# yewsiang/Transferable3D

Hardware: AMD Instinct MI355X
Metric: frustums/sec fwd+bwd (higher is better)
Workload: dtype f32

## Files before the change

### transferable3d_amd/csrc/poolbwd.hip

```cpp
#include "poolbwd_dev.h"

namespace {

__global__ __launch_bounds__(256) void k_pool_bwd_prep(const t3d_pool_bwd_prep_args p) {
  extern __shared__ __attribute__((aligned(16))) float smem[];
  pool_bwd_prep_body(p, smem, blockIdx.x, blockIdx.y, blockIdx.z);
}
__global__ __launch_bounds__(256) void k_pool_sparse_rows(const t3d_pool_sparse_rows_args p) {
  extern __shared__ __attribute__((aligned(16))) float smem[];
  pool_sparse_rows_body(p, smem, blockIdx.x, blockIdx.y);
}
template <class XT>
__global__ __launch_bounds__(256) void k_act_colsum(const t3d_act_colsum_args p) {
  extern __shared__ __attribute__((aligned(16))) float smem[];
  act_colsum_body<XT>(p, smem, blockIdx.x);
}
template <class XT>
__global__ __launch_bounds__(256) void k_pool_wgrad_finish(const t3d_pool_wgrad_finish_args p) {
  extern __shared__ __attribute__((aligned(16))) float smem[];
  pool_wgrad_finish_body<XT>(p, smem, blockIdx.x, blockIdx.y);
}

}

extern "C" int t3d_pool_bwd_prep(const t3d_pool_bwd_prep_args* a, t3d_stream_t stream) {
  const int rc = check_prep(a);
  if (rc != T3D_OK) return rc;
  T3D_LAUNCH(k_pool_bwd_prep, dim3(a->K / 32, a->K / 32, (a->N + PCH - 1) / PCH), dim3(256), PREP_LDS,
             static_cast<hipStream_t>(stream), *a);
  T3D_CHECK_LAUNCH();
  return T3D_OK;
}

extern "C" int t3d_pool_sparse_rows(const t3d_pool_sparse_rows_args* a, t3d_stream_t stream) {
  const int rc = check_sparse_rows(a);
  if (rc != T3D_OK) return rc;
  const size_t lds = sparse_rows_lds(a->N);
  static size_t allowed = 0;
  if (lds > 64 * 1024 && lds > allowed) {
    (void)hipFuncSetAttribute(reinterpret_cast<const void*>(k_pool_sparse_rows), hipFuncAttributeMaxDynamicSharedMemorySize,
                              (int)lds);
    allowed = lds;
  }
  const long M = (long)a->B * a->rows_per_frustum;
  T3D_LAUNCH(k_pool_sparse_rows, dim3(M / 128, a->K / SR_KC), dim3(256), lds, static_cast<hipStream_t>(stream), *a);
  T3D_CHECK_LAUNCH();
  return T3D_OK;
}

extern "C" int t3d_act_colsum(const t3d_act_colsum_args* a, t3d_stream_t stream) {
  const int rc = check_colsum(a);
  if (rc != T3D_OK) return rc;
  if (a->a.dtype == T3D_BF16) T3D_LAUNCH(k_act_colsum<bf16_t>, dim3(a->M / 128), dim3(256), COLSUM_LDS, static_cast<hipStream_t>(stream), *a);
  else T3D_LAUNCH(k_act_colsum<float>, dim3(a->M / 128), dim3(256), COLSUM_LDS, static_cast<hipStream_t>(stream), *a);
  T3D_CHECK_LAUNCH();
  return T3D_OK;
}

extern "C" int t3d_pool_wgrad_finish(const t3d_pool_wgrad_finish_args* a, t3d_stream_t stream) {
  const int rc = check_finish(a);
  if (rc != T3D_OK) return rc;
  const size_t lds = finish_lds(a->K);
  if (a->a.dtype == T3D_BF16) T3D_LAUNCH(k_pool_wgrad_finish<bf16_t>, dim3(a->K / FK, a->N / FN), dim3(256), lds, static_cast<hipStream_t>(stream), *a);
  else T3D_LAUNCH(k_pool_wgrad_finish<float>, dim3(a->K / FK, a->N / FN), dim3(256), lds, static_cast<hipStream_t>(stream), *a);
  T3D_CHECK_LAUNCH();
  return T3D_OK;
}
```

### transferable3d_amd/csrc/poolbwd_dev.h

```cpp
#pragma once
#include "common.h"

namespace {


constexpr int PCH = 128;

constexpr size_t PREP_LDS = (2 * 32 * (PCH + 1) + 2 * PCH) * sizeof(float);

__device__ __forceinline__ void pool_bwd_prep_body(const t3d_pool_bwd_prep_args& p, float* smem, int bi, int bj, int ch, int tid_ = -1) {
  float (*wi)[PCH + 1] = reinterpret_cast<float (*)[PCH + 1]>(smem);
  float (*wj)[PCH + 1] = reinterpret_cast<float (*)[PCH + 1]>(smem + 32 * (PCH + 1));
  float* v = smem + 2 * 32 * (PCH + 1);
  float* c0s = v + PCH;
  const int tid = tid_ < 0 ? (int)threadIdx.x : tid_, ti = tid >> 4, tj = tid & 15;
  const int n0 = ch * PCH;
  const bool edge = bj == 0;
  const float* c0 = p.coef;
  const float* c1 = p.coef + p.N;
  const float* c2 = p.coef + 2 * p.N;
#pragma unroll
  for (int q = 0; q < 4; ++q) {
    const int f = tid + 256 * q;
    const int r = f >> 5, c = (f & 31) * 4;
    const int n = min(n0 + c, p.N - 4);
    const bool ok = n0 + c < p.N;
    const float4 a = *reinterpret_cast<const float4*>(p.w + (size_t)(32 * bi + r) * p.N + n);
    const float4 b = *reinterpret_cast<const float4*>(p.w + (size_t)(32 * bj + r) * p.N + n);
    const float4 s1 = *reinterpret_cast<const float4*>(c1 + n);
    wi[r][c + 0] = ok ? a.x : 0.f; wi[r][c + 1] = ok ? a.y : 0.f; wi[r][c + 2] = ok ? a.z : 0.f; wi[r][c + 3] = ok ? a.w : 0.f;
    wj[r][c + 0] = ok ? b.x * s1.x : 0.f; wj[r][c + 1] = ok ? b.y * s1.y : 0.f;
    wj[r][c + 2] = ok ? b.z * s1.z : 0.f; wj[r][c + 3] = ok ? b.w * s1.w : 0.f;
  }
  if (tid < PCH) {
    const int n = min(n0 + tid, p.N - 1);
    const bool ok = n0 + tid < p.N;
    v[tid] = ok ? fmaf(p.bias ? p.bias[n] : 0.f, c1[n], c2[n]) : 0.f;
    c0s[tid] = ok ? c0[n] : 0.f;
  }
  __syncthreads();
  float a00 = 0.f, a01 = 0.f, a10 = 0.f, a11 = 0.f;
#pragma unroll 8
  for (int c = 0; c < PCH; ++c) {
    const float x0 = wi[ti][c], x1 = wi[ti + 16][c], y0 = wj[tj][c], y1 = wj[tj + 16][c];
    a00 = fmaf(x0, y0, a00); a01 = fmaf(x0, y1, a01);
    a10 = fmaf(x1, y0, a10); a11 = fmaf(x1, y1, a11);
  }
  float* ps = p.p_slabs + (size_t)ch * p.K * p.K;
  ps[(size_t)(32 * bi + ti) * p.K + 32 * bj + tj] = a00;
  ps[(size_t)(32 * bi + ti) * p.K + 32 * bj + tj + 16] = a01;
  ps[(size_t)(32 * bi + ti + 16) * p.K + 32 * bj + tj] = a10;
  ps[(size_t)(32 * bi + ti + 16) * p.K + 32 * bj + tj + 16] = a11;
  if (edge) {
    const int r = tid >> 3, q = tid & 7;
    float rc = 0.f;
#pragma unroll
    for (int c = q; c < PCH; c += 8) rc = fmaf(wi[r][c], v[c], rc);
    rc += __shfl_xor(rc, 4, 64);
    rc += __shfl_xor(rc, 2, 64);
    rc += __shfl_xor(rc, 1, 64);
    if (q == 0) p.rc_slabs[(size_t)ch * p.K + 32 * bi + r] = rc;
    const int k = tid & 31;
    if (p.wc != nullptr)
      for (int c = tid >> 5; c < PCH; c += 8)
        if (n0 + c < p.N) p.wc[(size_t)(n0 + c) * p.K + 32 * bi + k] = c0s[c] * wi[k][c];
  }
}

constexpr int SR_KC = 128;
constexpr int SR_UNROLL = 16;
constexpr int SR_PRE = 16;

__device__ __forceinline__ void pool_sparse_rows_body(const t3d_pool_sparse_rows_args& p, float* smem, int bx, int by) {
  float* tile = smem;
  int* lists = reinterpret_cast<int*>(smem + 128 * SR_KC);
  int* hitrow = lists + 4 * p.N;
  const int tid = threadIdx.x, lane = tid & 63, w = tid >> 6;
  const int row0 = bx * 128, kc0 = by * SR_KC;
  const int b = row0 / p.rows_per_frustum, rin0 = row0 - b * p.rows_per_frustum;
  for (int f = tid; f < 128 * SR_KC / 4; f += 256) reinterpret_cast<float4*>(tile)[f] = make_float4(0.f, 0.f, 0.f, 0.f);
  if (tid < 128) hitrow[tid] = 0;
  int* mine = lists + w * p.N;
  int cnt = 0;
  for (int nb = 0; nb < p.N; nb += 64 * SR_PRE) {
    int rr[SR_PRE];
#pragma unroll
    for (int q = 0; q < SR_PRE; ++q) {
      const int n = nb + 64 * q + lane;
      rr[q] = p.argidx[(size_t)b * p.N + min(n, p.N - 1)];
    }
#pragma unroll
    for (int q = 0; q < SR_PRE; ++q) {
      const int n = nb + 64 * q + lane;
      const int r = rr[q] - rin0;
      const bool hit = n < p.N && r >= 0 && r < 128 && (r & 3) == w;
      const unsigned long long m = __ballot(hit);
      if (hit) mine[cnt + __popcll(m & ((1ull << lane) - 1ull))] = n | (r << 16);
      cnt += __popcll(m);
    }
  }
  __syncthreads();
  for (int i0 = 0; i0 < cnt; i0 += SR_UNROLL) {
    float2 wv[SR_UNROLL];
    float g[SR_UNROLL];
    int rr[SR_UNROLL], en[SR_UNROLL];
#pragma unroll
    for (int u = 0; u < SR_UNROLL; ++u) en[u] = mine[min(i0 + u, cnt - 1)];
#pragma unroll
    for (int u = 0; u < SR_UNROLL; ++u) {
      const int n = en[u] & 0xffff;
      rr[u] = en[u] >> 16;
      g[u] = p.dpool[(size_t)b * p.N + n];
      wv[u] = *reinterpret_cast<const float2*>(p.wc + (size_t)n * p.K + kc0 + 2 * lane);
    }
#pragma unroll
    for (int u = 0; u < SR_UNROLL; ++u) {
      hitrow[rr[u]] = 1;
      g[u] = (i0 + u < cnt) ? g[u] : 0.f;
    }
#pragma unroll
    for (int u = 0; u < SR_UNROLL; ++u) {
      float2* t = reinterpret_cast<float2*>(tile + rr[u] * SR_KC + 2 * lane);
      float2 cur = *t;
      cur.x = fmaf(g[u], wv[u].x, cur.x);
      cur.y = fmaf(g[u], wv[u].y, cur.y);
      *t = cur;
    }
  }
  __syncthreads();
  const bool gated = p.row_live != nullptr;
  if (gated && by == 0 && tid < 128) p.row_live[row0 + tid] = hitrow[tid];
  for (int f = tid; f < 128 * SR_KC / 4; f += 256) {
    const int r = f / (SR_KC / 4), c4 = f % (SR_KC / 4);
    if (gated && !hitrow[r]) continue;
    *reinterpret_cast<float4*>(p.s + (size_t)(row0 + r) * p.K + kc0 + 4 * c4) = reinterpret_cast<const float4*>(tile)[f];
  }
}

__device__ __forceinline__ float act_elem(const t3d_act_src& s, size_t row, int k) {
  float v = ld_elem(s.x, row * s.ldx + s.coff + k, s.dtype);
  if (s.scale) v = fmaf(v, s.scale[k], s.shift[k]);
  if (s.relu) v = fmaxf(v, 0.f);
  return v;
}

constexpr size_t COLSUM_LDS = 256 * sizeof(float4);

template <class XT = float>
__device__ __forceinline__ void act_colsum_body(const t3d_act_colsum_args& p, float* smem, int bx) {
  float4* red = reinterpret_cast<float4*>(smem);
  const int tid = threadIdx.x;
  const int row0 = bx * 128;
  const int chunks = p.K / 4, c4 = tid % chunks, grp = tid / chunks, groups = 256 / chunks, rows = 128 / groups;
  float4 sc = make_float4(1.f, 1.f, 1.f, 1.f), sh = make_float4(0.f, 0.f, 0.f, 0.f);
  if (p.a.scale) {
    sc = *reinterpret_cast<const float4*>(p.a.scale + 4 * c4);
    sh = *reinterpret_cast<const float4*>(p.a.shift + 4 * c4);
  }
  const float floor_ = p.a.relu ? 0.f : -INFINITY;
  float4 acc = make_float4(0.f, 0.f, 0.f, 0.f);
  const size_t base = (size_t)(row0 + grp * rows) * p.a.ldx + p.a.coff + 4 * c4;
  constexpr int CSB = 16;
  for (int r0 = 0; r0 < rows; r0 += CSB) {
    typename Elem<XT>::V4 raw[CSB];
#pragma unroll
    for (int u = 0; u < CSB; ++u) raw[u] = Elem<XT>::ld4(p.a.x, base + (size_t)min(r0 + u, rows - 1) * p.a.ldx);
#pragma unroll
    for (int u = 0; u < CSB; ++u) {
      if (r0 + u < rows) {
        const float4 x = Elem<XT>::widen(raw[u]);
        acc.x += fmaxf(fmaf(x.x, sc.x, sh.x), floor_);
        acc.y += fmaxf(fmaf(x.y, sc.y, sh.y), floor_);
        acc.z += fmaxf(fmaf(x.z, sc.z, sh.z), floor_);
        acc.w += fmaxf(fmaf(x.w, sc.w, sh.w), floor_);
      }
    }
  }
  red[tid] = acc;
  __syncthreads();
  if (tid < chunks) {
    float4 t = red[tid];
    for (int g = 1; g < groups; ++g) {
      const float4 u = red[g * chunks + tid];
      t.x += u.x; t.y += u.y; t.z += u.z; t.w += u.w;
    }
    *reinterpret_cast<float4*>(p.part + (size_t)bx * p.K + 4 * tid) = t;
  }
}

constexpr int FK = 32, FN = 16, FB = 32;

inline size_t finish_lds(int K) {
  return ((size_t)FK * (K + 1) + (size_t)K * FN + FK * (FN + 1) + 2 * FB * FN) * sizeof(float);
}

template <class XT = float>
__device__ __forceinline__ void pool_wgrad_finish_body(const t3d_pool_wgrad_finish_args& p, float* smem, int bx, int by, int tid_ = -1) {
  float* gsm = smem;
  float* wsm = gsm + FK * (p.K + 1);
  float* gat = wsm + p.K * FN;
  float* dps = gat + FK * (FN + 1);
  int* ais = reinterpret_cast<int*>(dps + FB * FN);
  const int tid = tid_ < 0 ? (int)threadIdx.x : tid_;
  const int k0 = bx * FK, n0 = by * FN;
  const int ldg = p.K + 1;
  for (int f = tid; f < FK * p.K; f += 256) gsm[(f / p.K) * ldg + f % p.K] = p.g[(size_t)(k0 + f / p.K) * p.K + f % p.K];
  for (int f = tid; f < p.K * FN; f += 256) wsm[f] = p.w[(size_t)(f / FN) * p.N + n0 + f % FN];
  {
    const int k = tid & 31, q = tid >> 5;
    const float sc = p.a.scale ? p.a.scale[k0 + k] : 1.f, sh = p.a.scale ? p.a.shift[k0 + k] : 0.f;
    const float floor_ = p.a.relu ? 0.f : -INFINITY;
    const size_t xk = (size_t)(p.a.coff + k0 + k);
    float g0 = 0.f, g1 = 0.f;
    for (int b0 = 0; b0 < p.B; b0 += FB) {
      __syncthreads();
      for (int f = tid; f < FB * FN; f += 256) {
        const int b = b0 + f / FN;
        const bool ok = b < p.B;
        const size_t o = (size_t)min(b, p.B - 1) * p.N + n0 + f % FN;
        const int ai = p.argidx[o];
        const float dpv = p.dpool[o];
        dps[f] = (ok && ai >= 0) ? dpv : 0.f;
        ais[f] = max(ai, 0);
      }
      __syncthreads();
      float x0[FB], x1[FB];
#pragma unroll
      for (int bb = 0; bb < FB; ++bb) {
        const size_t rowbase = (size_t)min(b0 + bb, p.B - 1) * p.rows_per_frustum;
        x0[bb] = Elem<XT>::ld1(p.a.x, xk + (rowbase + ais[bb * FN + q]) * p.a.ldx);
        x1[bb] = Elem<XT>::ld1(p.a.x, xk + (rowbase + ais[bb * FN + q + 8]) * p.a.ldx);
      }
#pragma unroll
      for (int bb = 0; bb < FB; ++bb) {
        g0 = fmaf(dps[bb * FN + q], fmaxf(fmaf(x0[bb], sc, sh), floor_), g0);
        g1 = fmaf(dps[bb * FN + q + 8], fmaxf(fmaf(x1[bb], sc, sh), floor_), g1);
      }
    }
    gat[k * (FN + 1) + q] = g0;
    gat[k * (FN + 1) + q + 8] = g1;
  }
  __syncthreads();
  const int ti = tid >> 4, tj = tid & 15;
  float a0 = 0.f, a1 = 0.f;
#pragma unroll 8
  for (int j = 0; j < p.K; ++j) {
    const float wv = wsm[j * FN + tj];
    a0 = fmaf(gsm[ti * ldg + j], wv, a0);
    a1 = fmaf(gsm[(ti + 16) * ldg + j], wv, a1);
  }
  const int n = n0 + tj;
  const float c0 = p.coef[n], c1 = p.coef[p.N + n], c2 = p.coef[2 * p.N + n];
  const float bias = p.bias ? p.bias[n] : 0.f;
  const float ab0 = p.abar[k0 + ti], ab1 = p.abar[k0 + ti + 16];
  p.dw[(size_t)(k0 + ti) * p.N + n] = fmaf(c0, gat[ti * (FN + 1) + tj], fmaf(c1, fmaf(ab0, bias, a0), ab0 * c2));
  p.dw[(size_t)(k0 + ti + 16) * p.N + n] = fmaf(c0, gat[(ti + 16) * (FN + 1) + tj], fmaf(c1, fmaf(ab1, bias, a1), ab1 * c2));
}



inline bool pool_act_ok(const t3d_act_src& a, int K) {
  return a.x != nullptr && a.coff + K <= a.ldx && (a.scale == nullptr || a.shift != nullptr) && a.sub == nullptr;
}
inline int check_prep(const t3d_pool_bwd_prep_args* a) {
  if (!a || !a->w || !a->coef || !a->p_slabs || !a->rc_slabs) return T3D_ERR_ARG;
  if (a->K <= 0 || a->K % 32 || a->N <= 0 || a->N % 4) return T3D_ERR_SHAPE;
  return T3D_OK;
}
inline size_t sparse_rows_lds(int N) { return (size_t)128 * SR_KC * sizeof(float) + ((size_t)4 * N + 128) * sizeof(int); }
inline int check_sparse_rows(const t3d_pool_sparse_rows_args* a) {
  if (!a || !a->argidx || !a->dpool || !a->wc || !a->s) return T3D_ERR_ARG;
  if (a->B <= 0 || a->N <= 0 || a->N > 65535 || a->K % SR_KC || a->rows_per_frustum % T3D_TILE_ROWS ||
      a->rows_per_frustum > 32767 || sparse_rows_lds(a->N) > 160 * 1024)
    return T3D_ERR_SHAPE;
  return T3D_OK;
}
inline int check_colsum(const t3d_act_colsum_args* a) {
  if (!a || !a->part || !pool_act_ok(a->a, a->K)) return T3D_ERR_ARG;
  if (a->M <= 0 || a->M % T3D_TILE_ROWS || (a->K != 64 && a->K != 128 && a->K != 256) || a->a.ldx % 4 || a->a.coff % 4)
    return T3D_ERR_SHAPE;
  return T3D_OK;
}
inline int check_finish(const t3d_pool_wgrad_finish_args* a) {
  if (!a || !a->argidx || !a->dpool || !a->coef || !a->w || !a->g || !a->abar || !a->dw || !pool_act_ok(a->a, a->K))
    return T3D_ERR_ARG;
  if (a->K <= 0 || a->K % FK || a->K > 256 || a->N <= 0 || a->N % FN || a->B <= 0) return T3D_ERR_SHAPE;
  return T3D_OK;
}

}
```

Before: 27660.

## Rewrite sparse-row pooling backward as counting-sort row lists with segmented accumulation

Replaces the default sparse-rows kernel with a version that buckets hit points by destination row via wave-ballot ranking, a prefix scan over per-wave row counts, and a compact sorted (offset|row, grad) list. Waves then split the sorted list into balanced row-aligned ranges and do a segmented FMA accumulation with double-buffered prefetch of weight rows, writing only touched rows and zeroing empty ones directly. This targets the zero-fill of the full LDS tile and the per-row scanning cost of the old scheme. The old tile kernel stays reachable through an environment variable, and a new shape check guards the 32-bit byte offset packing.

```diff
diff --git a/transferable3d_amd/csrc/poolbwd.hip b/transferable3d_amd/csrc/poolbwd.hip
--- a/transferable3d_amd/csrc/poolbwd.hip
+++ b/transferable3d_amd/csrc/poolbwd.hip
@@ -1,3 +1,4 @@
+#include <stdlib.h>
 #include "poolbwd_dev.h"
 
 namespace {
@@ -9,6 +10,10 @@
 __global__ __launch_bounds__(256) void k_pool_sparse_rows(const t3d_pool_sparse_rows_args p) {
   extern __shared__ __attribute__((aligned(16))) float smem[];
   pool_sparse_rows_body(p, smem, blockIdx.x, blockIdx.y);
+}
+__global__ __launch_bounds__(256) void k_pool_sparse_rows_tile(const t3d_pool_sparse_rows_args p) {
+  extern __shared__ __attribute__((aligned(16))) float smem[];
+  pool_sparse_rows_tile_body(p, smem, blockIdx.x, blockIdx.y);
 }
 template <class XT>
 __global__ __launch_bounds__(256) void k_act_colsum(const t3d_act_colsum_args p) {
@@ -36,14 +41,17 @@
   const int rc = check_sparse_rows(a);
   if (rc != T3D_OK) return rc;
   const size_t lds = sparse_rows_lds(a->N);
-  static size_t allowed = 0;
-  if (lds > 64 * 1024 && lds > allowed) {
-    (void)hipFuncSetAttribute(reinterpret_cast<const void*>(k_pool_sparse_rows), hipFuncAttributeMaxDynamicSharedMemorySize,
-                              (int)lds);
-    allowed = lds;
+  const char* e_ = getenv("T3D_SPARSE_ROWS");
+  const bool tile = e_ && atoi(e_) == 0;
+  static size_t allowed[2] = {0, 0};
+  if (lds > 64 * 1024 && lds > allowed[tile]) {
+    (void)hipFuncSetAttribute(tile ? reinterpret_cast<const void*>(k_pool_sparse_rows_tile) : reinterpret_cast<const void*>(k_pool_sparse_rows),
+                              hipFuncAttributeMaxDynamicSharedMemorySize, (int)lds);
+    allowed[tile] = lds;
   }
   const long M = (long)a->B * a->rows_per_frustum;
-  T3D_LAUNCH(k_pool_sparse_rows, dim3(M / 128, a->K / SR_KC), dim3(256), lds, static_cast<hipStream_t>(stream), *a);
+  if (tile) T3D_LAUNCH(k_pool_sparse_rows_tile, dim3(M / 128, a->K / SR_KC), dim3(256), lds, static_cast<hipStream_t>(stream), *a);
+  else T3D_LAUNCH(k_pool_sparse_rows, dim3(M / 128, a->K / SR_KC), dim3(256), lds, static_cast<hipStream_t>(stream), *a);
   T3D_CHECK_LAUNCH();
   return T3D_OK;
 }
diff --git a/transferable3d_amd/csrc/poolbwd_dev.h b/transferable3d_amd/csrc/poolbwd_dev.h
--- a/transferable3d_amd/csrc/poolbwd_dev.h
+++ b/transferable3d_amd/csrc/poolbwd_dev.h
@@ -70,8 +70,194 @@
 constexpr int SR_KC = 128;
 constexpr int SR_UNROLL = 16;
 constexpr int SR_PRE = 16;
+constexpr int SRL_PRE = 8;
+constexpr int SRL_U = 16;
+constexpr int SRL_OFF = 128 * SR_KC;
+constexpr int SRL_LIST = SRL_OFF + 130;
+
+__device__ __forceinline__ void srl_issue(int2 (&en)[SRL_U], float2 (&wv)[SRL_U], const int2* ent, const char* wcb, unsigned lane8,
+                                          int i0, int e) {
+#pragma unroll
+  for (int u = 0; u < SRL_U; ++u) en[u] = ent[min(i0 + u, e - 1)];
+#pragma unroll
+  for (int u = 0; u < SRL_U; ++u) wv[u] = *reinterpret_cast<const float2*>(wcb + (((unsigned)en[u].x & ~511u) | lane8));
+}
+
+template <bool TAIL>
+__device__ __forceinline__ void srl_consume(const int2 (&en)[SRL_U], const float2 (&wv)[SRL_U], float* rows, int rem, int& prev, float2& acc) {
+#pragma unroll
+  for (int u = 0; u < SRL_U; ++u) {
+    if (!TAIL || u < rem) {
+      const int row = en[u].x & 127;
+      const float g = __int_as_float(en[u].y);
+      const bool fresh = row != prev;
+      acc.x = fmaf(g, wv[u].x, fresh ? 0.f : acc.x);
+      acc.y = fmaf(g, wv[u].y, fresh ? 0.f : acc.y);
+      *reinterpret_cast<float2*>(rows + row * SR_KC) = acc;
+      prev = row;
+    }
+  }
+}
 
 __device__ __forceinline__ void pool_sparse_rows_body(const t3d_pool_sparse_rows_args& p, float* smem, int bx, int by) {
+  int* cnt = reinterpret_cast<int*>(smem);
+  int* stage = cnt + 4 * 128;
+  float* dstage = reinterpret_cast<float*>(stage + p.N);
+  int* off = cnt + SRL_OFF;
+  int2* list = reinterpret_cast<int2*>(cnt + SRL_LIST);
+  const int tid = threadIdx.x, lane = tid & 63;
+  const int w = __builtin_amdgcn_readfirstlane(tid >> 6);
+  const int row0 = bx * 128, kc0 = by * SR_KC;
+  const int b = row0 / p.rows_per_frustum, rin0 = row0 - b * p.rows_per_frustum;
+  const bool gated = p.row_live != nullptr;
+  const int cpw = ((p.N + 63) / 64 + 3) / 4;
+  const int n_lo = min(w * cpw * 64, p.N), n_hi = min(n_lo + cpw * 64, p.N);
+  int* mycnt = cnt + w * 128;
+  mycnt[lane] = 0;
+  mycnt[lane + 64] = 0;
+  for (int nb = n_lo; nb < n_hi; nb += 64 * SRL_PRE) {
+    int rr[SRL_PRE];
+    float dd[SRL_PRE];
+#pragma unroll
+    for (int q = 0; q < SRL_PRE; ++q) {
+      const size_t o = (size_t)b * p.N + min(nb + 64 * q + lane, p.N - 1);
+      rr[q] = p.argidx[o];
+      dd[q] = p.dpool[o];
+    }
+#pragma unroll
+    for (int q = 0; q < SRL_PRE; ++q) {
+      const int n = nb + 64 * q + lane;
+      if (nb + 64 * q < n_hi) {
+        const int r = rr[q] - rin0;
+        const bool hit = n < n_hi && r >= 0 && r < 128;
+        unsigned long long rem = __ballot(hit);
+        int rank = 0, tot = 0, lead = lane;
+        while (rem) {
+          const int l = __ffsll(rem) - 1;
+          const int rl = __builtin_amdgcn_readlane(r, l);
+          const bool me = hit && r == rl;
+          const unsigned long long m = __ballot(me);
+          const int below = __builtin_amdgcn_mbcnt_hi((unsigned)(m >> 32), __builtin_amdgcn_mbcnt_lo((unsigned)m, 0u));
+          rank = me ? below : rank;
+          tot = me ? __popcll(m) : tot;
+          lead = me ? l : lead;
+          rem &= ~m;
+        }
+        int old = 0;
+        if (hit && lead == lane) {
+          old = mycnt[r];
+          mycnt[r] = old + tot;
+        }
+        old = __shfl(old, lead, 64);
+        if (n < n_hi) {
+          stage[n] = hit ? (r << 16) | (old + rank) : -1;
+          dstage[n] = dd[q];
+        }
+      }
+    }
+  }
+  __syncthreads();
+  if (w == 0) {
+    int c0[4], c1[4];
+#pragma unroll
+    for (int q = 0; q < 4; ++q) {
+      const int2 c = *reinterpret_cast<const int2*>(cnt + q * 128 + 2 * lane);
+      c0[q] = c.x;
+      c1[q] = c.y;
+    }
+    const int t0 = c0[0] + c0[1] + c0[2] + c0[3], t1 = c1[0] + c1[1] + c1[2] + c1[3];
+    int incl = t0 + t1;
+#pragma unroll
+    for (int d = 1; d < 64; d <<= 1) {
+      const int v = __shfl_up(incl, d, 64);
+      if (lane >= d) incl += v;
+    }
+    const int excl = incl - (t0 + t1);
+    *reinterpret_cast<int2*>(off + 2 * lane) = make_int2(excl, excl + t0);
+    if (lane == 63) off[128] = incl;
+    int run0 = excl, run1 = excl + t0;
+#pragma unroll
+    for (int q = 0; q < 4; ++q) {
+      *reinterpret_cast<int2*>(cnt + q * 128 + 2 * lane) = make_int2(run0, run1);
+      run0 += c0[q];
+      run1 += c1[q];
+    }
+    if (gated && by == 0) {
+      p.row_live[row0 + 2 * lane] = t0 > 0;
+      p.row_live[row0 + 2 * lane + 1] = t1 > 0;
+    }
+  }
+  __syncthreads();
+  for (int n = n_lo + lane; n < n_hi; n += 64) {
+    const int e = stage[n];
+    if (e >= 0) {
+      const int r = e >> 16, d = mycnt[r] + (e & 0xffff);
+      list[d] = make_int2(n * p.K * 4 | r, __float_as_int(dstage[n]));
+    }
+  }
+  __syncthreads();
+  float* srow = p.s + (size_t)row0 * p.K + kc0 + 2 * lane;
+  if (!gated) {
+    const int rz = 32 * w + (lane & 31);
+    unsigned long long z = __ballot(lane < 32 && off[rz] == off[rz + 1]);
+    while (z) {
+      const int l = __ffsll(z) - 1;
+      *reinterpret_cast<float2*>(srow + (size_t)(32 * w + l) * p.K) = make_float2(0.f, 0.f);
+      z &= z - 1;
+    }
+  }
+  const int H = off[128];
+  int se[2];
+#pragma unroll
+  for (int j = 0; j < 2; ++j) {
+    const int bound = (w + j) * H / 4;
+    int v = H;
+    if (w + j < 4 && bound < H) {
+      const int r = list[bound].x & 127;
+      v = off[r] == bound ? bound : off[r + 1];
+    }
+    se[j] = __builtin_amdgcn_readfirstlane(v);
+  }
+  const int s = se[0], e = se[1];
+  if (s >= e) return;
+  const char* wcb = reinterpret_cast<const char*>(p.wc + kc0);
+  const unsigned lane8 = 8u * lane;
+  float* rows = smem + 2 * lane;
+  int prev = -1;
+  float2 acc = make_float2(0.f, 0.f);
+  int2 ea[SRL_U], eb[SRL_U];
+  float2 wa[SRL_U], wb[SRL_U];
+  srl_issue(ea, wa, list, wcb, lane8, s, e);
+  for (int i0 = s; i0 < e; i0 += 2 * SRL_U) {
+    srl_issue(eb, wb, list, wcb, lane8, i0 + SRL_U, e);
+    if (e - i0 >= SRL_U) srl_consume<false>(ea, wa, rows, SRL_U, prev, acc);
+    else srl_consume<true>(ea, wa, rows, e - i0, prev, acc);
+    srl_issue(ea, wa, list, wcb, lane8, i0 + 2 * SRL_U, e);
+    if (e - i0 >= 2 * SRL_U) srl_consume<false>(eb, wb, rows, SRL_U, prev, acc);
+    else srl_consume<true>(eb, wb, rows, e - i0 - SRL_U, prev, acc);
+  }
+  const int first = __builtin_amdgcn_readfirstlane(list[s].x & 127), last = __builtin_amdgcn_readfirstlane(list[e - 1].x & 127);
+  for (int rb = first; rb <= last; rb += 64) {
+    const int r = min(rb + lane, 127);
+    unsigned long long m = __ballot(rb + lane <= last && off[r + 1] > off[r]);
+    while (m) {
+      int r4[4];
+#pragma unroll
+      for (int j = 0; j < 4; ++j) {
+        r4[j] = rb + __ffsll(m) - 1;
+        const unsigned long long mm = m & (m - 1);
+        m = (j < 3 && mm == 0) ? m : mm;
+      }
+      float2 v[4];
+#pragma unroll
+      for (int j = 0; j < 4; ++j) v[j] = *reinterpret_cast<const float2*>(rows + r4[j] * SR_KC);
+#pragma unroll
+      for (int j = 0; j < 4; ++j) *reinterpret_cast<float2*>(srow + (size_t)r4[j] * p.K) = v[j];
+    }
+  }
+}
+
+__device__ __forceinline__ void pool_sparse_rows_tile_body(const t3d_pool_sparse_rows_args& p, float* smem, int bx, int by) {
   float* tile = smem;
   int* lists = reinterpret_cast<int*>(smem + 128 * SR_KC);
   int* hitrow = lists + 4 * p.N;
@@ -271,7 +457,7 @@
 inline int check_sparse_rows(const t3d_pool_sparse_rows_args* a) {
   if (!a || !a->argidx || !a->dpool || !a->wc || !a->s) return T3D_ERR_ARG;
   if (a->B <= 0 || a->N <= 0 || a->N > 65535 || a->K % SR_KC || a->rows_per_frustum % T3D_TILE_ROWS ||
-      a->rows_per_frustum > 32767 || sparse_rows_lds(a->N) > 160 * 1024)
+      a->rows_per_frustum > 32767 || sparse_rows_lds(a->N) > 160 * 1024 || (long)a->N * a->K * 4 > 0x7fffffffL)
     return T3D_ERR_SHAPE;
   return T3D_OK;
 }
```

New measurement: 27840 (median of 6 runs). About the same (+0.7%).
